# mit-han-lab/litepose

Measured on AMD Instinct MI355X. Metric: images/sec end-to-end (backbone+deconv+AE-group), LitePose-XS@256 b64, higher is better.
Workload: dtype f32

## Files before the change

### include/litepose_amd.h

```cpp
#ifndef LITEPOSE_AMD_H
#define LITEPOSE_AMD_H

#include <stddef.h>
#include <stdint.h>

#ifdef __cplusplus
extern "C" {
#endif

typedef enum lp_status {
    LP_OK = 0,
    LP_ERR_INVALID_ARG = -1,
    LP_ERR_UNKNOWN_KEY = -2,
    LP_ERR_SHAPE = -3,
    LP_ERR_MISSING_WEIGHT = -4,
    LP_ERR_NOT_FINALIZED = -5,
    LP_ERR_WORKSPACE = -6,
    LP_ERR_HIP = -7,
    LP_ERR_UNSUPPORTED = -8,
    LP_ERR_CAPACITY = -9
} lp_status;

const char* lp_last_error(void);
const char* lp_version(void);
// ... 221 lines not shown
                      float push_factor, float pull_factor, const float* d_g_heat, const float* d_g_push,
                      const float* d_g_pull, float* d_grad, void* stream);

size_t lp_bn_workspace_bytes(int N, int C, int HW);
int lp_bn_forward(const float* d_x, const float* d_gamma, const float* d_beta, float* d_running, const float* d_res,
                  float* d_y, double* d_stat, int N, int C, int HW, int act, int training, double momentum, double eps,
                  void* d_workspace, size_t workspace_bytes, void* stream);
int lp_bn_backward(const float* d_grad_y, const float* d_x, const float* d_gamma, const float* d_beta, const double* d_stat,
                   float* d_grad_x, float* d_grad_gamma, float* d_grad_beta, int N, int C, int HW, int act,
                   void* d_workspace, size_t workspace_bytes, void* stream);

#define LP_BN_SYNC_MAX_WORLD 64
int lp_bn_sync_stats(const float* d_x, int N, int C, int HW, double* d_row, void* d_workspace, size_t workspace_bytes,
                     void* stream);
int lp_bn_sync_forward(const float* d_x, const float* d_gamma, const float* d_beta, float* d_running, const float* d_res,
                       float* d_y, double* d_stat, const double* d_rows, int W, int N, int C, int HW, int act,
                       double momentum, double eps, void* stream);
int lp_bn_sync_backward_stats(const float* d_grad_y, const float* d_x, const float* d_gamma, const float* d_beta,
                              const double* d_stat, int N, int C, int HW, int act, double* d_row, void* d_workspace,
                              size_t workspace_bytes, void* stream);
int lp_bn_sync_backward(const float* d_grad_y, const float* d_x, const float* d_gamma, const float* d_beta,
                        const double* d_stat, const double* d_rows, int W, int rank, int N, int C, int HW, int act,
                        float* d_grad_x, float* d_grad_gamma, float* d_grad_beta, void* stream);

int lp_pw_tile_choice(int N, int Ca, int Cb, int Cout, int HW, int has_res);
#define LP_PW_WGRAD_SLICE 1024

#define LP_MBT_NONE 0
#define LP_MBT_TILE 1
#define LP_MBT_STRIP 2
#define LP_MBT_S2 3
int lp_mbt_form(int N, int Cin, int Cexp, int Cout, int H, int W, int K, int S, int has_res, int mode, int mode_s2,
                int mode_strip, int cus);
size_t lp_pw_forward_workspace_bytes(int Cin, int Cout);
int lp_pw_forward(const float* d_x, const float* d_w, float* d_y, int N, int Cin, int Cout, int HW, void* d_workspace,
                  size_t workspace_bytes, void* stream);
size_t lp_pw_backward_workspace_bytes(int N, int Cin, int Cout, int HW, int want_x, int want_w);
int lp_pw_backward(const float* d_grad_y, const float* d_x, const float* d_w, float* d_grad_x, float* d_grad_w, int N,
                   int Cin, int Cout, int HW, void* d_workspace, size_t workspace_bytes, void* stream);

#define LP_DW_WGRAD_SLICE 8
size_t lp_dw_forward_workspace_bytes(int C, int K);
int lp_dw_forward(const float* d_x, const float* d_w, float* d_y, int N, int C, int H, int W, int K, int S,
                  void* d_workspace, size_t workspace_bytes, void* stream);
size_t lp_dw_backward_workspace_bytes(int N, int C, int H, int W, int K, int S, int want_w);
int lp_dw_backward(const float* d_grad_y, const float* d_x, const float* d_w, float* d_grad_x, float* d_grad_w, int N,
                   int C, int H, int W, int K, int S, void* d_workspace, size_t workspace_bytes, void* stream);

#define LP_STEM_WGRAD_SLICE 2048
int lp_stem_forward(const float* d_x, const float* d_w, float* d_y, int N, int H, int W, void* stream);
size_t lp_stem_backward_workspace_bytes(int N, int H, int W);
int lp_stem_backward(const float* d_grad_y, const float* d_x, float* d_grad_w, int N, int H, int W, void* d_workspace,
                     size_t workspace_bytes, void* stream);

#define LP_DECONV_WGRAD_SLICE 1024
size_t lp_deconv_forward_workspace_bytes(int Ca, int Cb, int Cout);
int lp_deconv_forward(const float* d_xa, const float* d_wa, const float* d_xb, const float* d_wb, float* d_y, int N,
                      int Ca, int Cb, int Cout, int h, int w, void* d_workspace, size_t workspace_bytes, void* stream);
size_t lp_deconv_backward_workspace_bytes(int N, int Ca, int Cb, int Cout, int h, int w, int want_x, int want_w);
int lp_deconv_backward(const float* d_grad_y, const float* d_xa, const float* d_wa, const float* d_xb, const float* d_wb,
                       float* d_grad_xa, float* d_grad_xb, float* d_grad_wa, float* d_grad_wb, int N, int Ca,
                       int Cb, int Cout, int h, int w, void* d_workspace, size_t workspace_bytes, void* stream);

#define LP_CONV_WGRAD_SLICE 1024
size_t lp_conv_workspace_bytes(int N, int Ca, int Cb, int Cout, int H, int W, int K, int S, int ups);
int lp_conv_forward(const float* d_xa, const float* d_wa, const float* d_xb, const float* d_wb, const float* d_bias,
// ... 61 lines not shown
```

### litepose_amd/_native.py

```python
import ctypes as C
import os

import torch

_HERE = os.path.dirname(os.path.abspath(__file__))
LIB_PATH = os.path.join(_HERE, 'lib', 'liblitepose_amd.so')
if os.environ.get('LP_NATIVE_FLAVOUR'):
    LIB_PATH = os.path.join(_HERE, 'lib', 'liblitepose_amd_%s.so' % os.environ['LP_NATIVE_FLAVOUR'])

LP_MAX_STAGES, LP_MAX_BLOCKS, LP_MAX_DECONV = 8, 32, 4


class LpArch(C.Structure):
    _fields_ = [
        ('input_channel', C.c_int32), ('num_stages', C.c_int32),
        ('num_blocks', C.c_int32 * LP_MAX_STAGES), ('stride', C.c_int32 * LP_MAX_STAGES),
        ('channel', C.c_int32 * LP_MAX_STAGES),
        ('expand', (C.c_int32 * LP_MAX_BLOCKS) * LP_MAX_STAGES),
        ('kernel', (C.c_int32 * LP_MAX_BLOCKS) * LP_MAX_STAGES),
        ('num_deconv', C.c_int32), ('deconv_filters', C.c_int32 * LP_MAX_DECONV),
        ('head_channels', C.c_int32 * LP_MAX_DECONV),
        ('plain_head', C.c_int32),
        ('family', C.c_int32),
        ('upconv_kernel', C.c_int32),
# ... 103 lines not shown
                            vp, vp, vp, sz, vp]),
    'lp_kpt_eval': (i32, [vp, vp, vp, i32, i32, i32, i32, i32, vp, vp, vp, vp, vp, vp, i32, C.POINTER(C.c_double),
                          C.POINTER(C.c_double), i32, C.POINTER(C.c_double), i32, i32, vp, vp, vp, vp, vp, vp, vp]),
    'lp_draw_poses': (i32, [vp, i32, i32, i32, vp, vp, i32, i32, i32, C.POINTER(C.c_int32), i32,
                            C.POINTER(C.c_uint8), i32, i32, i32, vp]),
    'lp_draw_poses_v': (i32, [vp, sz, vp, i32, vp, vp, i32, i32, i32, C.POINTER(C.c_int32), i32,
                              C.POINTER(C.c_uint8), i32, i32, i32, vp]),
    'lp_draw_pass_prims': (i32, []),
    'lp_preprocess': (i32, [vp, i32, i32, C.POINTER(C.c_double), i32, i32, C.POINTER(C.c_float),
                            C.POINTER(C.c_float), vp, vp, vp]),
    'lp_preprocess_batch': (i32, [vp, i32, i32, i32, C.POINTER(C.c_double), i32, i32, C.POINTER(C.c_float),
                                  C.POINTER(C.c_float), vp, vp, vp]),
    'lp_warp_invert': (i32, [C.POINTER(C.c_double), C.POINTER(C.c_double)]),
    'lp_preprocess_batch_v': (i32, [vp, sz, vp, i32, i32, i32, C.POINTER(C.c_float), C.POINTER(C.c_float), vp, vp,
                                    vp]),
    'lp_augment_batch_v': (i32, [vp, sz, vp, i32, i32, i32, C.POINTER(C.c_float), C.POINTER(C.c_float), vp, vp, vp]),
    'lp_target_maps': (i32, [vp, i64, vp, vp, i32, i32, i32, C.POINTER(C.c_int32), vp, i32, C.c_double, i32, i32, vp, vp,
                             vp]),
    'lp_target_masks': (i32, [vp, sz, vp, i32, i32, vp, vp]),
    'lp_pose_loss_workspace_bytes': (sz, [i32, i32, i32]),
    'lp_pose_loss': (i32, [vp, i32, i32, i32, i32, i32, vp, vp, vp, i32, i32, C.c_float, C.c_float, C.c_float, vp, vp, vp,
                           vp, sz, vp]),
    'lp_pose_loss_grad': (i32, [vp, i32, i32, i32, i32, i32, vp, vp, vp, i32, i32, C.c_float, C.c_float, C.c_float, vp, vp,
                                vp, vp, vp]),
    'lp_bn_workspace_bytes': (sz, [i32, i32, i32]),
    'lp_bn_forward': (i32, [vp, vp, vp, vp, vp, vp, vp, i32, i32, i32, i32, i32, C.c_double, C.c_double, vp, sz, vp]),
    'lp_bn_backward': (i32, [vp, vp, vp, vp, vp, vp, vp, vp, i32, i32, i32, i32, vp, sz, vp]),
    'lp_bn_sync_stats': (i32, [vp, i32, i32, i32, vp, vp, sz, vp]),
    'lp_bn_sync_forward': (i32, [vp, vp, vp, vp, vp, vp, vp, vp, i32, i32, i32, i32, i32, C.c_double, C.c_double, vp]),
    'lp_bn_sync_backward_stats': (i32, [vp, vp, vp, vp, vp, i32, i32, i32, i32, vp, vp, sz, vp]),
    'lp_bn_sync_backward': (i32, [vp, vp, vp, vp, vp, vp, i32, i32, i32, i32, i32, i32, vp, vp, vp, vp]),
    'lp_pw_tile_choice': (i32, [i32, i32, i32, i32, i32, i32]),
    'lp_mbt_form': (i32, [i32] * 13),
    'lp_pw_forward_workspace_bytes': (sz, [i32, i32]),
    'lp_pw_forward': (i32, [vp, vp, vp, i32, i32, i32, i32, vp, sz, vp]),
    'lp_pw_backward_workspace_bytes': (sz, [i32, i32, i32, i32, i32, i32]),
    'lp_pw_backward': (i32, [vp, vp, vp, vp, vp, i32, i32, i32, i32, vp, sz, vp]),
    'lp_dw_forward_workspace_bytes': (sz, [i32, i32]),
    'lp_dw_forward': (i32, [vp, vp, vp, i32, i32, i32, i32, i32, i32, vp, sz, vp]),
    'lp_dw_backward_workspace_bytes': (sz, [i32, i32, i32, i32, i32, i32, i32]),
    'lp_dw_backward': (i32, [vp, vp, vp, vp, vp, i32, i32, i32, i32, i32, i32, vp, sz, vp]),
    'lp_stem_forward': (i32, [vp, vp, vp, i32, i32, i32, vp]),
    'lp_stem_backward_workspace_bytes': (sz, [i32, i32, i32]),
    'lp_stem_backward': (i32, [vp, vp, vp, i32, i32, i32, vp, sz, vp]),
    'lp_deconv_forward_workspace_bytes': (sz, [i32, i32, i32]),
    'lp_deconv_forward': (i32, [vp, vp, vp, vp, vp, i32, i32, i32, i32, i32, i32, vp, sz, vp]),
    'lp_deconv_backward_workspace_bytes': (sz, [i32, i32, i32, i32, i32, i32, i32, i32]),
    'lp_deconv_backward': (i32, [vp, vp, vp, vp, vp, vp, vp, vp, vp, i32, i32, i32, i32, i32, i32, vp, sz, vp]),
    'lp_conv_workspace_bytes': (sz, [i32] * 9),
    'lp_conv_forward': (i32, [vp, vp, vp, vp, vp, vp] + [i32] * 9 + [vp, sz, vp]),
    'lp_conv_backward': (i32, [vp] * 10 + [i32] * 9 + [vp, sz, vp]),
    'lp_optim_launches': (i32, [i32, C.POINTER(i64)]),
    'lp_optim_adam': (i32, [i32, C.POINTER(vp), C.POINTER(vp), C.POINTER(vp), C.POINTER(vp), C.POINTER(i64), vp, vp,
                            C.c_double, C.c_double, C.c_double, C.c_double, vp]),
    'lp_optim_sgd': (i32, [i32, C.POINTER(vp), C.POINTER(vp), C.POINTER(vp), C.POINTER(i64), vp, C.c_double, C.c_double,
                           i32, vp]),
    'lp_subnet_gather': (i32, [vp, i32, vp, i64, vp]),
    'lp_subnet_scatter_grad': (i32, [vp, i32, vp, i64, vp, i64, vp]),
    'lp_train_resize': (i32, [vp, vp, i32, i32, i32, i32, i32, i32, i32, C.POINTER(C.c_int32), C.POINTER(vp), C.POINTER(vp),
                              C.POINTER(vp), C.POINTER(vp), C.POINTER(vp), C.POINTER(vp), vp]),
    'lp_stream_abort_capture': (i32, [vp]),
    'lp_final_preds': (i32, [vp, vp, i32, i32, i32, i32, C.POINTER(C.c_double), C.POINTER(C.c_double),
                             i32, i32, vp]),
    'lp_final_preds_coef': (i32, [C.POINTER(C.c_double), C.POINTER(C.c_double), i32, i32, C.POINTER(C.c_double)]),
    'lp_final_preds_v': (i32, [vp, vp, i32, i32, i32, i32, vp, vp]),
}
# ... 38 lines not shown
```

### litepose_amd/csrc/engine.cpp

```cpp
#include <hip/hip_runtime.h>

#include <cmath>
#include <cstdio>
#include <cstdint>
#include <cstring>
#include <map>
#include <string>
#include <vector>

#include "../../include/litepose_amd.h"
#include "kernels.h"
#include "plan.h"

using namespace lp_plan;

namespace {

thread_local std::string g_err;
int fail(int code, const std::string& msg) {
    g_err = msg;
    return code;
}
#define HIP_OK(expr)                                                                   \
    do {                                                                               \
// ... 3 lines not shown
    } while (0)

static_assert(ACT_NONE == lp::ACT_NONE && ACT_RELU == lp::ACT_RELU && ACT_RELU6 == lp::ACT_RELU6, "plan.h restates lp::Act");

const char* storage_name(const Net* n) { return n->storage == LP_STORAGE_F16 ? "f16" : "bf16"; }

}

struct lp_net : lp_plan::Net {
    bool finalized = false;
    float* d_weights = nullptr;
    std::vector<char*> last_buf;
    int lastN = 0, lastH = 0, lastW = 0;
    bool profiling = false;
    std::vector<hipEvent_t> events;
    struct ProfEntry { std::string name, kernel; int64_t bytes, flops; int ev0, ev1; int64_t flops_valu; lp::LaunchNote launch; };
    std::vector<ProfEntry> prof_entries;
    int prof_ev = 0;
    static constexpr int MAX_SIDE = 8;
    hipStream_t side[MAX_SIDE] = {};
    hipEvent_t ev_fork = nullptr, ev_join[MAX_SIDE] = {};
    int nstreams = 0;
    int opt_mb16 = 1;
    int opt_mb16_run = 1;
    int opt_mb16_min = 48;
    int opt_mbt = 1, opt_mbt_s2 = 1;
    int opt_mbt_strip = 1;
    int opt_mbconv2 = 1;
    int opt_mbtb = 1, opt_mbtb_s2 = 1;
    int opt_pw3d = 1;
    int opt_mbtd = 1;
    int opt_headb = 1;
    int opt_headfuse = 1;
    int opt_dwt = 2;
    int opt_stem = 1;
    int opt_diag_dwpw = 0;
    struct OptEntryT { const char* key; int lo, hi; int lp_net::*field; };
    static const std::vector<OptEntryT>& options();
    std::vector<char> last_stored;
    struct CalibLayer { std::string bn; int C, div; size_t off; };
    struct Calib {
        lp_net* raw = nullptr;
        std::vector<CalibLayer> layers;
        std::map<std::string, int> index;
        std::vector<float> h_bn;
        float* d_bn = nullptr;
        double momentum = 0.1;
        int64_t steps = 0;
        bool uploaded = false;
    };
    Calib* calib = nullptr;
};

namespace {

size_t buf_elems(const lp_net* n, int b, int N, int H, int W, size_t esz) {
    const int d = n->bufs.div[b];
    const size_t f = (size_t)N * n->bufs.ch[b] * (H / d) * (W / d), q = 256 / esz;
    return (f + q - 1) / q * q;
}
size_t buf_floats(const lp_net* n, int b, int N, int H, int W) { return buf_elems(n, b, N, H, W, sizeof(float)); }

size_t buf_bytes(const lp_net* n, int b, int N, int H, int W) {
    const size_t esz = n->storage != LP_STORAGE_F32 ? sizeof(uint16_t) : sizeof(float);
    return buf_elems(n, b, N, H, W, esz) * esz;
}
// ... 327 lines not shown
}

int rule_dwpw3(const Part& c, size_t i) {
    const lp_net* n = c.n;
    const Op& o = n->ops[i];
    if (!(o.type == OP_DW && o.K == 3 && o.S == 1 && o.act == lp::ACT_RELU6 && i + 1 < n->ops.size())) return 0;
    const Op& pw = n->ops[i + 1];
    if (!(pw.type == OP_PW && pw.inA == o.out && pw.inB < 0 && pw.res < 0 && pw.act == lp::ACT_NONE && pw.has_bias)) return 0;
    const Planes pl = planes(c, o);
    const float* Wt = c.Wt;
    return lp::launch_dwpw(c.f(o.inA), Wt + o.w_off, Wt + o.b_off, Wt + pw.w_off, Wt + pw.b_off, nullptr, c.f(pw.out), c.NB,
                           o.Ca, pl.ih, pl.iw, o.K, o.S, pw.Cout, c.s, n->opt_diag_dwpw) ? 2 : 0;
}

int rule_head(const Part& c, size_t i) {
    const lp_net* n = c.n;
    const std::vector<Op>& ops = n->ops;
    const Op& o = ops[i];
    if (!(n->opt_headfuse && o.type == OP_DW && o.S == 1 && o.act == lp::ACT_RELU && i + 1 < ops.size())) return 0;
    const Op& a = ops[i + 1];
    const Op *d2 = nullptr, *pw = nullptr;
    if (o.K == 5 && a.type == OP_PW && a.inA == o.out && a.inB < 0 && a.res < 0 && a.act == lp::ACT_NONE &&
        (a.out == n->out0_buf || a.out == n->out1_buf))
        pw = &a;
    else if (i + 2 < ops.size() && a.type == OP_DW && ops[i + 2].type == OP_PW && ops[i + 2].inA == o.out &&
             ops[i + 2].inB == a.out && a.S == 1 && o.K == a.K && a.act == lp::ACT_RELU)
        d2 = &a, pw = &ops[i + 2];
    else
        return 0;
    const Planes pl = planes(c, o);
    const float* Wt = c.Wt;
    if (!lp::launch_headfuse(c.f(o.inA), o.Ca, d2 ? c.f(d2->inA) : nullptr, d2 ? d2->Ca : 0,
                             o.wpair_off ? Wt + o.wpair_off : nullptr, d2 && d2->wpair_off ? Wt + d2->wpair_off : nullptr,
                             Wt + pw->w_off, c.f(pw->out), c.NB, pl.oh, pl.ow, o.K, pw->Cout, c.s))
        return 0;
    return d2 ? 3 : 2;
}

const Rule F32_RULES[] = {{rule_mb16, block_name, nullptr}, {rule_mbt, block_name, nullptr}, {rule_stem3, stem_name, nullptr},
                          {rule_dwpw3, dwpw3_name, nullptr}, {rule_head, head_name, nullptr}};

int launch_op_f32(const Part& c, size_t i) {
    const lp_net* n = c.n;
    const Op& o = n->ops[i];
    const Planes pl = planes(c, o);
    const int ih = pl.ih, iw = pl.iw, oh = pl.oh, ow = pl.ow, NB = c.NB;
    const float* Wt = c.Wt;
    hipStream_t s = c.s;
    switch (o.type) {
        case OP_STEM:
            lp::launch_stem(c.x, Wt + o.w_off, Wt + o.b_off, c.f(o.out), NB, c.H, c.W, c.flip_from, c.x_batch, s);
            break;
        case OP_DW:
            lp::launch_dw(c.f(o.inA), Wt + o.w_off, Wt + o.wdup_off, Wt + o.b_off, c.f(o.out), NB, o.Ca, ih, iw, o.K, o.S,
                          o.act, s);
            break;
        case OP_PW:
            lp::launch_pw(c.f(o.inA), o.Ca, o.inB >= 0 ? c.f(o.inB) : nullptr, o.Cb, Wt + o.w_off,
                          o.has_bias ? Wt + o.b_off : nullptr, o.res >= 0 ? c.f(o.res) : nullptr, c.f(o.out), NB, oh * ow,
                          o.Cout, o.act, s, o.ws_off ? Wt + o.ws_off : nullptr, n->opt_pw3d);
            break;
        case OP_DECONV: {
            float* inB = o.inB >= 0 ? c.f(o.inB) : nullptr;
            if (o.w3_off && deconv4_enabled() && o.w4_off &&
                lp::launch_deconv4x3(c.f(o.inA), o.Ca, inB, o.Cb, Wt + o.w4_off, Wt + o.b3_off, c.f(o.out), NB, ih, iw,
                                     o.Cout, s)) {
            } else if (o.w3_off && deconv4_enabled())
// ... 418 lines not shown
        n->storage = storage;
        n->finalized = false;
        n->last_buf.clear();
    }
    return LP_OK;
}

int lp_net_get_storage(const lp_net* n) { return n ? n->storage : LP_ERR_INVALID_ARG; }

int lp_round16(const float* h_src, float* h_dst, int64_t count, int storage) {
    if ((!h_src || !h_dst) && count > 0) return fail(LP_ERR_INVALID_ARG, "null argument");
    if (storage != LP_STORAGE_BF16 && storage != LP_STORAGE_F16)
        return fail(LP_ERR_INVALID_ARG, "storage must be LP_STORAGE_BF16 or LP_STORAGE_F16");
    for (int64_t i = 0; i < count; ++i) h_dst[i] = round16(storage, h_src[i]);
    return LP_OK;
}

typedef lp_net::OptEntryT OptEntry;
const std::vector<OptEntry>& lp_net::options() {
    static const std::vector<OptEntry> t = {
        {"mb16", 0, 1, &lp_net::opt_mb16},
        {"mb16_run", 0, 1, &lp_net::opt_mb16_run},
        {"mb16_min", 0, 65536, &lp_net::opt_mb16_min},
        {"mbt", 0, 3, &lp_net::opt_mbt},
        {"mbt_s2", 0, 1, &lp_net::opt_mbt_s2},
        {"mbt_strip", 0, 2, &lp_net::opt_mbt_strip},
        {"mbconv2", 0, 1, &lp_net::opt_mbconv2},
        {"mbtb", 0, 1, &lp_net::opt_mbtb},
        {"mbtb_s2", 0, 1, &lp_net::opt_mbtb_s2},
        {"mbtd", 0, 1, &lp_net::opt_mbtd},
        {"pw3d", 0, 2, &lp_net::opt_pw3d},
        {"headb", 0, 1, &lp_net::opt_headb},
        {"headfuse", 0, 1, &lp_net::opt_headfuse},
        {"dwt", 0, 2, &lp_net::opt_dwt},
        {"stem", 0, 1, &lp_net::opt_stem},
        {"diag_dwpw", 0, 2, &lp_net::opt_diag_dwpw},
    };
    return t;
}

int lp_net_set_option(lp_net* n, const char* key, int value) {
    if (!n || !key) return fail(LP_ERR_INVALID_ARG, "null argument");
    for (const OptEntry& e : lp_net::options())
        if (!strcmp(key, e.key)) {
            if (value < e.lo || value > e.hi) return fail(LP_ERR_INVALID_ARG, std::string("option ") + key + ": value out of range");
#ifndef LP_DIAG_BUILD
            if (e.field == &lp_net::opt_diag_dwpw && value != 0)
                return fail(LP_ERR_UNSUPPORTED, "option diag_dwpw: the self-checking dwpw_kernel exists only in the diagnostics "
                                                "flavour of the library (python -m litepose_amd.build --flavour diag, "
                                                "LP_NATIVE_FLAVOUR=diag)");
#endif
            n->*(e.field) = value;
            return LP_OK;
        }
    return fail(LP_ERR_UNKNOWN_KEY, std::string("unknown option ") + key);
}

int lp_net_get_option(const lp_net* n, const char* key) {
    if (!n || !key) return fail(LP_ERR_INVALID_ARG, "null argument");
    for (const OptEntry& e : lp_net::options())
        if (!strcmp(key, e.key)) return n->*(e.field);
    return fail(LP_ERR_UNKNOWN_KEY, std::string("unknown option ") + key);
}

int lp_diag_read(uint32_t* h_words, int cap_words, int clear) {
    const int n = lp::dwpw_diag_read(h_words, cap_words, clear != 0);
// ... 66 lines not shown
```

### litepose_amd/csrc/kernels.h

```cpp
#pragma once
#include <hip/hip_runtime.h>
#include <stdint.h>

namespace lp {

enum Act { ACT_NONE = 0, ACT_RELU = 1, ACT_RELU6 = 2 };

bool uses_scratch(const void* kernel_fn);

bool kernel_ready(const void* kernel_fn, size_t dyn_lds);
bool kernel_allow_lds(const void* kernel_fn, size_t dyn_lds);

extern thread_local const char* last_kernel_tag;

struct LaunchNote { int grid = 0, block = 0, lds = 0, wgs_per_cu = 0; };
extern thread_local LaunchNote last_launch;
extern thread_local bool launch_notes;
void note_launch(const void* fn, dim3 grid, dim3 block, size_t lds);
#define LP_LAUNCH(kern, grid, block, lds, stream, ...)                                                   \
    do {                                                                                                 \
        if (lp::launch_notes) lp::note_launch(reinterpret_cast<const void*>(kern), grid, block, lds);    \
        hipLaunchKernelGGL(kern, grid, block, lds, stream, __VA_ARGS__);                                 \
    } while (0)

#ifdef LP_CLAIM_CU
#define LP_OWN_CU() asm volatile("; own the CU: whole register budget, no co-resident waves" ::: "v255")
#else
#define LP_OWN_CU() ((void)0)
#endif

void launch_stem(const float* x, const float* w, const float* b, float* out,
                 int N, int H, int W, int flip_from, int x_batch, hipStream_t s);

bool launch_stem3(const float* x, const float* w0t, const float* b0, const float* w1t, const float* b1,
                  const float* w2t, const float* b2, float* out, int N, int H, int W, int c0, int flip_from,
                  int x_batch, hipStream_t s);

bool launch_stem3b(const float* x, const float* w0t, const float* b0, const float* w1t, const float* b1,
                   const float* w2t, const float* b2, void* out, int N, int H, int W, int c0, int flip_from,
                   int x_batch, hipStream_t s, bool f16 = false);

void launch_dw(const float* in, const float* w, const float* wdup, const float* b, float* out,
               int N, int C, int H, int W, int K, int S, int act, hipStream_t s);

void launch_pw(const float* inA, int Ca, const float* inB, int Cb,
               const float* wp, const float* b, const float* res, float* out,
               int N, int HW, int Cout, int act, hipStream_t s, const void* wsplit = nullptr, int pw3d_mode = 1);
struct PwTile { int NB, PXV; };
PwTile pw_tile_choice(int N, int Ca, int Cb, int Cout, int HW, bool has_res);

bool launch_dwpw(const float* in, const float* wdw, const float* bdw, const float* wp, const float* bias,
                 const float* res, float* out, int N, int C, int H, int W, int K, int S, int Cout,
                 hipStream_t s, int diag = 0);
int dwpw_diag_read(unsigned* host, int cap_words, bool clear);

bool launch_headfuse(const float* inA, int Ca, const float* inB, int Cb, const float* wpairA, const float* wpairB,
                     const float* wp, float* out, int N, int H, int W, int K, int Cout, hipStream_t s);

bool launch_mbconv(const float* x, const float* w1p, const float* b1f, const float* wdw,
                   const float* bdw, const float* w2p, const float* b2f, const float* res, float* out,
                   int N, int Cin, int Cexp, int Cout, int H, int W, int K, int S, hipStream_t s,
                   const float* wdw_pair = nullptr, const void* w1_split = nullptr, const void* wdw_rows = nullptr,
                   int mbconv2 = 1);

constexpr int MB16_MAX_RUN = 10;
struct Mb16Run {
    const void* w1s[MB16_MAX_RUN];
    const float* b1f[MB16_MAX_RUN];
    const void* wrow[MB16_MAX_RUN];
    const void* w2s[MB16_MAX_RUN];
    const float* b2f[MB16_MAX_RUN];
    float* out[MB16_MAX_RUN];
    int nblocks;
};
bool mb16_supported(int Cin, int Cexp, int Cout, int H, int W, int K, int S, bool res);
bool launch_mb16(const float* x, const Mb16Run& run, bool res, int N, int Cin, int Cexp, int Cout, int H, int W,
                 int K, int S, hipStream_t s);

bool launch_mbt(const float* x, const void* w1s, const float* b1f, const void* wrow, const void* w2s,
                const float* b2f, const float* res, float* out, int N, int Cin, int Cexp, int Cout, int H, int W,
                int K, int S, hipStream_t s, int mode = 1, int mode_s2 = 1, int mode_strip = 1);
enum MbtKind { MBT_NONE = 0, MBT_TILE = 1, MBT_STRIP = 2, MBT_S2 = 3 };
struct MbtForm { int kind = MBT_NONE, CK = 0, NMT = 0; bool RES = false; };
MbtForm mbt_form(int N, int Cin, int Cexp, int Cout, int H, int W, int K, int S, bool has_res, int mode, int mode_s2,
                 int mode_strip, int cus);

void launch_deconv_pair(const float* inA, int Ca, const float* inB, int Cb,
                        const float* w, const float* b, float* out,
                        int N, int h, int w_, int Cout, hipStream_t s);

// ... 215 lines not shown
```

### litepose_amd/csrc/layer_api.cpp

```cpp
#include <hip/hip_runtime.h>

#include "../../include/litepose_amd.h"
#include "kernels.h"

extern "C" void lp_set_error_(const char* msg);

namespace {
int fail(int code, const char* msg) {
    lp_set_error_(msg);
    return code;
}
bool al16(const void* p) { return ((uintptr_t)p & 15) == 0; }
bool big(long long v) { return v > 0x7fffff00LL; }
size_t frag_floats(int M, int K) { return (size_t)((M + 31) / 32) * ((K + 1) / 2) * 64; }
size_t bias_floats(int M) { return (size_t)((M + 31) / 32) * 32; }
bool dw_shape_ok(int K, int S) { return (K == 3 || K == 5 || K == 7) && (S == 1 || S == 2); }
}

extern "C" {

size_t lp_bn_workspace_bytes(int N, int C, int HW) {
    if (N < 1 || C < 1 || HW < 1 || C > 65535 || big((long long)N * HW) || big((long long)C * HW)) return 0;
    return lp::bn_partial_doubles(N, C, HW) * sizeof(double);
}
// ... 98 lines not shown
                        const double* d_stat, const double* d_rows, int W, int rank, int N, int C, int HW, int act,
                        float* d_grad_x, float* d_grad_gamma, float* d_grad_beta, void* stream) {
    if (int rc = sync_check(N, C, HW, act, W, rank)) return rc;
    if (!d_grad_y || !d_x || !d_gamma || !d_beta || !d_stat || !d_rows || !d_grad_x || !d_grad_gamma || !d_grad_beta)
        return fail(LP_ERR_INVALID_ARG, "null argument");
    if (!al16(d_grad_y) || !al16(d_x) || !al16(d_grad_x) || !al8(d_stat) || !al8(d_rows))
        return fail(LP_ERR_INVALID_ARG, "grad_y, x and grad_x must be 16-byte, stat and rows 8-byte aligned");
    lp::launch_bn_sync_bwd(d_grad_y, d_x, d_gamma, d_beta, d_stat, d_rows, W, rank, d_grad_x, d_grad_gamma,
                           d_grad_beta, N, C, HW, act, (hipStream_t)stream);
    if (hipGetLastError() != hipSuccess) return fail(LP_ERR_HIP, "bn_sync_backward launch failed");
    return LP_OK;
}

static int pw_check(int N, int Cin, int Cout, int HW) {
    if (N < 1 || Cin < 1 || Cout < 1 || HW < 1) return fail(LP_ERR_INVALID_ARG, "N, Cin, Cout and HW must be positive");
    if (Cin > 65535 || Cout > 65535 || big((long long)N * HW) || big((long long)Cin * HW) || big((long long)Cout * HW))
        return fail(LP_ERR_UNSUPPORTED, "channels must be <= 65535, N * HW and C * HW at most 2^31 - 256");
    return LP_OK;
}

int lp_pw_tile_choice(int N, int Ca, int Cb, int Cout, int HW, int has_res) {
    if (N < 1 || Ca < 1 || Cb < 0 || Cout < 1 || HW < 1) return fail(LP_ERR_INVALID_ARG, "N, Ca, Cout and HW must be positive, Cb non-negative");
    const lp::PwTile t = lp::pw_tile_choice(N, Ca, Cb, Cout, HW, has_res != 0);
    return t.NB * 16 + t.PXV;
}

int lp_mbt_form(int N, int Cin, int Cexp, int Cout, int H, int W, int K, int S, int has_res, int mode, int mode_s2,
                int mode_strip, int cus) {
    if (N < 1 || Cin < 1 || Cexp < 1 || Cout < 1 || H < 1 || W < 1 || K < 1 || S < 1)
        return fail(LP_ERR_INVALID_ARG, "N, Cin, Cexp, Cout, H, W, K and S must be positive");
    const lp::MbtForm f = lp::mbt_form(N, Cin, Cexp, Cout, H, W, K, S, has_res != 0, mode, mode_s2, mode_strip, cus);
    if (f.kind == lp::MBT_NONE) return LP_MBT_NONE;
    return f.kind + 16 * f.CK + 256 * f.NMT + (f.RES ? 4096 : 0);
}

size_t lp_pw_forward_workspace_bytes(int Cin, int Cout) {
    if (Cin < 1 || Cout < 1 || Cin > 65535 || Cout > 65535) return 0;
    return (frag_floats(Cout, Cin) + bias_floats(Cout)) * sizeof(float);
}

int lp_pw_forward(const float* d_x, const float* d_w, float* d_y, int N, int Cin, int Cout, int HW, void* d_workspace,
                  size_t workspace_bytes, void* stream) {
    if (int rc = pw_check(N, Cin, Cout, HW)) return rc;
    if (!d_x || !d_w || !d_y) return fail(LP_ERR_INVALID_ARG, "null argument");
    if (!al16(d_x) || !al16(d_y)) return fail(LP_ERR_INVALID_ARG, "x and y must be 16-byte aligned");
    if (!d_workspace || workspace_bytes < lp_pw_forward_workspace_bytes(Cin, Cout)) return fail(LP_ERR_WORKSPACE, "pw workspace too small");
    if (!al16(d_workspace)) return fail(LP_ERR_WORKSPACE, "pw workspace must be 16-byte aligned");
    hipStream_t s = (hipStream_t)stream;
    float* wp = (float*)d_workspace;
    float* zb = wp + frag_floats(Cout, Cin);
    lp::launch_pw_pack(d_w, Cout, Cin, false, wp, zb, s);
    lp::launch_pw(d_x, Cin, nullptr, 0, wp, zb, nullptr, d_y, N, HW, Cout, lp::ACT_NONE, s);
    if (hipGetLastError() != hipSuccess) return fail(LP_ERR_HIP, "pw_forward launch failed");
    return LP_OK;
}

size_t lp_pw_backward_workspace_bytes(int N, int Cin, int Cout, int HW, int want_x, int want_w) {
    if (N < 1 || Cin < 1 || Cout < 1 || HW < 1 || Cin > 65535 || Cout > 65535 || big((long long)N * HW)) return 0;
    size_t fl = 0;
    if (want_x) fl += frag_floats(Cin, Cout) + bias_floats(Cin);
    if (want_w) fl += (size_t)lp::pw_wgrad_slices((long)N * HW) * Cout * Cin;
    return fl * sizeof(float);
}

int lp_pw_backward(const float* d_grad_y, const float* d_x, const float* d_w, float* d_grad_x, float* d_grad_w, int N,
                   int Cin, int Cout, int HW, void* d_workspace, size_t workspace_bytes, void* stream) {
// ... 328 lines not shown
```

### litepose_amd/csrc/net_kernels.hip

```cpp
#include "kernels.h"
#include "fused_common.h"
#include "split3.h"

#include <cstdio>
#include <cstdlib>
#include <type_traits>
#include <utility>

namespace lp {

thread_local const char* last_kernel_tag = "";
thread_local LaunchNote last_launch;
thread_local bool launch_notes = false;

void note_launch(const void* fn, dim3 grid, dim3 block, size_t lds) {
    int per_cu = 0;
    const int threads = (int)(block.x * block.y * block.z);
    if (hipOccupancyMaxActiveBlocksPerMultiprocessor(&per_cu, fn, threads, lds) != hipSuccess) per_cu = 0;
    last_launch.grid = (int)((long)grid.x * grid.y * grid.z);
    last_launch.block = threads;
    last_launch.lds = (int)lds;
    last_launch.wgs_per_cu = per_cu;
}

// ... 1269 lines not shown
        const unsigned z = 0;
        if (hipMemcpyToSymbol(HIP_SYMBOL(lp_dwpw_diag_log), &z, 4, 0, hipMemcpyHostToDevice) != hipSuccess) return -1;
    }
    return (int)n;
#endif
}

bool launch_dwpw(const float* in, const float* wdw, const float* bdw, const float* wp, const float* bias,
                 const float* res, float* out, int N, int C, int H, int W, int K, int S, int Cout,
                 hipStream_t s, int diag) {
    if ((K != 7 && K != 3) || (C & 31) || (W & 3) || Cout > 96) return false;
    if (K == 3 && (S != 1 || Cout > 32)) return false;
    {
        const int OHt = (H + 2 * (K / 2) - K) / S + 1, OWt = (W + 2 * (K / 2) - K) / S + 1;
        if ((long)OHt * OWt < 4096) return false;
    }
    const int nb = (Cout + 31) / 32;
    if (K == 3) {
        launch_dwpw_t<3, 1, 1>(in, wdw, bdw, wp, bias, res, out, N, C, H, W, Cout, s, diag);
        return true;
    }
#define LP_F(SV, NBV) launch_dwpw_t<7, SV, NBV>(in, wdw, bdw, wp, bias, res, out, N, C, H, W, Cout, s)
    if (S == 1) { if (nb == 1) LP_F(1, 1); else if (nb == 2) LP_F(1, 2); else LP_F(1, 3); }
    else { if (nb == 1) LP_F(2, 1); else if (nb == 2) LP_F(2, 2); else LP_F(2, 3); }
#undef LP_F
    return true;
}


__device__ __forceinline__ int quad_row_of_lane(int lane) {
    return (int)((0xFDCE5764B98A1320ull >> (4 * (lane >> 2))) & 15);
}

template <int NB, bool DUAL>
__global__ __launch_bounds__(256) void headfuse_kernel(const float* __restrict__ inA, int Ca,
                                                       const float* __restrict__ inB, int Cb,
                                                       const float* __restrict__ wpairA,
                                                       const float* __restrict__ wpairB,
                                                       const float* __restrict__ wp,
                                                       float* __restrict__ out, int H, int W, int tilesX, int tilesY,
                                                       int Cout, int xcd_remap) {
    constexpr int K = 5;
    constexpr int HALO = K / 2;
    constexpr int IH = 16 + K - 1;
    constexpr int QPR = 6;
    constexpr int RS = 13;
    constexpr int TILE_SLOTS = IH * RS;
    extern __shared__ __attribute__((aligned(16))) float smem[];
    const int C = DUAL ? Ca + Cb : Ca;
    float* slab = smem;
    const int lane = threadIdx.x & 63;
    const int wave = __builtin_amdgcn_readfirstlane(threadIdx.x >> 6);
    f32x4* tile = reinterpret_cast<f32x4*>(smem + 16 * 256) + wave * TILE_SLOTS;
    const int unit = xcd_remap ? xcd_contiguous_id(blockIdx.x, gridDim.x) : blockIdx.x;
    const int tq = unit / tilesX;
    const int tx = unit - tq * tilesX;
    const int n = tq / tilesY;
    const int ty = tq - n * tilesY;
    const int ix0 = tx * 16 - 4, iy0 = ty * 16 - HALO;
    constexpr int NQ = IH * QPR, NLD = (NQ + 63) / 64;
    const int row = quad_row_of_lane(lane), strip = lane & 3;
    const int half = lane >> 5, pl = lane & 31;
    const int KP = C >> 1;
    const int cblocks = (Cout + 31) >> 5;
    int st_off[NLD], st_lds[NLD];
#pragma unroll
    for (int i = 0; i < NLD; ++i) {
        const int e = lane + 64 * i;
        const int r = e / QPR, q = e - r * QPR;
        const int iy = iy0 + r, ix = ix0 + 4 * q;
        const bool ok = e < NQ && iy >= 0 && iy < H && ix >= 0 && ix < W;
        st_off[i] = ok ? iy * W + ix : -1;
        st_lds[i] = e < NQ ? r * RS + 2 * q : -1;
    }
    const long HW = (long)H * W;
    const float* imgA = inA + (long)n * Ca * HW;
    const float* imgB = DUAL ? inB + (long)n * Cb * HW : imgA;
    float afr[NB][32];
#pragma unroll
    for (int i = 0; i < NB; ++i)
#pragma unroll
        for (int kp = 0; kp < 32; ++kp)
            afr[i][kp] = wp[((long)min(i, cblocks - 1) * KP + min(kp, KP - 1)) * 64 + lane];
    f32x4 pre[2][NLD];
    auto issue = [&](int cp) {
        const int c = 2 * cp;
        const float* plane = (!DUAL || c < Ca) ? imgA + (long)c * HW : imgB + (long)(c - Ca) * HW;
#pragma unroll
        for (int h2 = 0; h2 < 2; ++h2)
#pragma unroll
            for (int i = 0; i < NLD; ++i) {
                f32x4 v = *reinterpret_cast<const f32x4*>(plane + h2 * HW + max(st_off[i], 0));
                if (st_off[i] < 0) v = f32x4{0.f, 0.f, 0.f, 0.f};
                pre[h2][i] = v;
            }
    };
    issue(wave);
    f32x16 acc[NB][2];
#pragma unroll
    for (int i = 0; i < NB; ++i)
#pragma unroll
        for (int v = 0; v < 2; ++v)
#pragma unroll
            for (int r = 0; r < 16; ++r) acc[i][v][r] = 0.f;
    const float* bsrc = slab + half * 256 + wave * 64 + 2 * pl;
    auto kpair_mfma = [&](int kp) {
        const f32x2 bv = *reinterpret_cast<const f32x2*>(bsrc + (kp & 7) * 512);
#pragma unroll
        for (int i = 0; i < NB; ++i) {
            acc[i][0] = __builtin_amdgcn_mfma_f32_32x32x2f32(afr[i][kp], bv[0], acc[i][0], 0, 0, 0);
            acc[i][1] = __builtin_amdgcn_mfma_f32_32x32x2f32(afr[i][kp], bv[1], acc[i][1], 0, 0, 0);
        }
    };
    const int NR = (KP + 3) >> 2;
#pragma unroll
    for (int u = 0; u < 8; ++u) {
        if (u >= NR) break;
        const int cp = wave + 4 * u;
        const bool has = cp < KP;
        const int c = 2 * cp;
        f32x2 dacc[4];
        f32x2 dbias = {0.f, 0.f};
        const float* wc = wpairA;
        if (has) {
#pragma unroll
            for (int i = 0; i < NLD; ++i)
                if (st_lds[i] >= 0) {
                    const f32x4 a = pre[0][i], b = pre[1][i];
                    tile[st_lds[i]] = f32x4{a[0], b[0], a[1], b[1]};
                    tile[st_lds[i] + 1] = f32x4{a[2], b[2], a[3], b[3]};
                }
            __builtin_amdgcn_fence(__ATOMIC_RELEASE, "wavefront");
            __builtin_amdgcn_wave_barrier();
            __builtin_amdgcn_fence(__ATOMIC_ACQUIRE, "wavefront");
            if (cp + 4 < KP) issue(cp + 4);
            wc = (!DUAL || c < Ca) ? wpairA + (long)cp * (K * K + 1) * 2 : wpairB + (long)(cp - (Ca >> 1)) * (K * K + 1) * 2;
            dbias = f32x2{wc[2 * K * K], wc[2 * K * K + 1]};
#pragma unroll
            for (int i = 0; i < 4; ++i) dacc[i] = DUAL ? dbias : f32x2{0.f, 0.f};
        }
#pragma unroll
        for (int ky = 0; ky < K; ++ky) {
            if (has) {
                const f32x4* lr = tile + (row + ky) * RS + 2 * strip;
                f32x2 v[12];
#pragma unroll
                for (int q = 0; q < 6; ++q) {
                    const f32x4 tt = lr[q];
                    v[2 * q] = f32x2{tt[0], tt[1]};
                    v[2 * q + 1] = f32x2{tt[2], tt[3]};
                }
#pragma unroll
                for (int kx = 0; kx < K; ++kx) {
                    const f32x2 w2 = {wc[2 * (ky * K + kx)], wc[2 * (ky * K + kx) + 1]};
#pragma unroll
                    for (int i = 0; i < 4; ++i) dacc[i] = __builtin_elementwise_fma(v[(4 - HALO) + kx + i], w2, dacc[i]);
                }
            }
            if (u > 0 && ky < 4) {
                const int kp = 4 * (u - 1) + ky;
                if (kp < KP) {
                    __builtin_amdgcn_sched_barrier(0);
                    kpair_mfma(kp);
                    __builtin_amdgcn_sched_barrier(0);
                }
            }
        }
        if (has) {
            f32x4 o0, o1;
#pragma unroll
            for (int i = 0; i < 4; ++i) {
                o0[i] = fmaxf(DUAL ? dacc[i][0] : dacc[i][0] + dbias[0], 0.f);
                o1[i] = fmaxf(DUAL ? dacc[i][1] : dacc[i][1] + dbias[1], 0.f);
            }
            *reinterpret_cast<f32x4*>(slab + (2 * (cp & 7)) * 256 + row * 16 + strip * 4) = o0;
            *reinterpret_cast<f32x4*>(slab + (2 * (cp & 7) + 1) * 256 + row * 16 + strip * 4) = o1;
        }
        __syncthreads();
    }
#pragma unroll
    for (int u = 0; u < 8; ++u)
        if (u == NR - 1) {
#pragma unroll
            for (int j = 0; j < 4; ++j)
                if (4 * u + j < KP) kpair_mfma(4 * u + j);
        }
    const int p0 = wave * 64 + 2 * pl;
    const int oy = ty * 16 + (p0 >> 4), ox = tx * 16 + (p0 & 15);
    if (oy >= H || ox >= W) return;
#pragma unroll
    for (int i = 0; i < NB; ++i) {
        if (i >= cblocks) break;
        const int cob = i * 32 + 4 * half;
#pragma unroll
        for (int r = 0; r < 16; ++r) {
            const int co = cob + (r & 3) + 8 * (r >> 2);
            if (co < Cout)
                *reinterpret_cast<f32x2*>(out + ((long)n * Cout + co) * HW + (long)oy * W + ox) =
                    f32x2{acc[i][0][r], acc[i][1][r]};
        }
    }
}

bool launch_headfuse(const float* inA, int Ca, const float* inB, int Cb, const float* wpairA, const float* wpairB,
                     const float* wp, float* out, int N, int H, int W, int K, int Cout, hipStream_t s) {
    const int C = Ca + Cb;
    const bool dual = inB != nullptr;
    if (!wpairA || (dual ? (!wpairB || (Cb & 1)) : Cb != 0) || K != 5 || (Ca & 1) || C > 64 || (W & 15) || (H & 15) ||
        Cout > 64 || (long)H * W < 4096)
        return false;
    const int tilesX = W / 16, tilesY = H / 16;
    const int grid = N * tilesX * tilesY;
    const size_t lds = (size_t)(16 * 256 + 4 * (16 + 5 - 1) * 13 * 4) * sizeof(float);
    static_assert((16 * 256 + 4 * (16 + 5 - 1) * 13 * 4) * sizeof(float) <= 64 * 1024,
                  "33 KB: below the default dynamic-LDS limit, no per-device attribute call needed (ADVICE r05)");
    last_kernel_tag = "headfuse_kernel";
#define LP_HF(NBV, DV) LP_LAUNCH((headfuse_kernel<NBV, DV>), dim3(grid), dim3(256), lds, s, inA, Ca, inB, Cb, \
                                 wpairA, wpairB, wp, out, H, W, tilesX, tilesY, Cout, xcd_remap_mode())
    if (dual) { if (Cout <= 32) LP_HF(1, true); else LP_HF(2, true); }
    else { if (Cout <= 32) LP_HF(1, false); else LP_HF(2, false); }
#undef LP_HF
    return true;
}

constexpr int MB_RS = 24, MB_ROWS = 22, MB_PLANE = MB_RS * MB_ROWS;

constexpr int MB2_RS = 26, MB2_PAIR = MB_ROWS * MB2_RS * 2;

__device__ __forceinline__ int mb2_row_of_lane(int lane) {
    return (int)((0xFDCE5764B98A1320ull >> (4 * (lane >> 2))) & 15);
}

template <bool RES>
__global__ __launch_bounds__(256, 2) void mbconv_kernel(
    const float* __restrict__ x,
    const float* __restrict__ w1p,
    const float* __restrict__ b1f,
    const float* __restrict__ wdwp,
    const float* __restrict__ bdw,
    const float* __restrict__ w2p,
    const float* __restrict__ b2f,
    float* __restrict__ out,
    int Cin, int Cexp, int Cout, int H, int W, int tilesX, int tilesY, int xcd_remap) {
    extern __shared__ __attribute__((aligned(16))) float E[];
    const int lane = threadIdx.x & 63;
    const int wave = __builtin_amdgcn_readfirstlane(threadIdx.x >> 6);
    const int half = lane >> 5, pl = lane & 31;
    const int unit = xcd_remap ? xcd_contiguous_id(blockIdx.x, gridDim.x) : blockIdx.x;
    const int tq = unit / tilesX;
    const int tx = unit - tq * tilesX;
    const int n = tq / tilesY;
    const int ty = tq - n * tilesY;
    const int x0 = tx * 16, y0 = ty * 16;
// ... 1083 lines not shown
```

Before: 23610.

## Add block-layout depthwise path to fused head kernel with register row streaming

Adds a BLK variant of the fused head kernel. Each lane computes a 2x2 output block for one channel pair, streaming input rows from LDS into registers so each row load serves two output rows. The MFMA pointwise step is interleaved under every row, and the NB==1 case gets a higher occupancy bound. It is on by default and falls back to the old variant if the new one spills to scratch. In exchange it adds template instantiations, a different slab write pattern with a swizzle, and some register pressure risk.

```diff
diff --git a/include/litepose_amd.h b/include/litepose_amd.h
--- a/include/litepose_amd.h
+++ b/include/litepose_amd.h
@@ -277,6 +277,9 @@
 #define LP_MBT_S2 3
 int lp_mbt_form(int N, int Cin, int Cexp, int Cout, int H, int W, int K, int S, int has_res, int mode, int mode_s2,
                 int mode_strip, int cus);
+#define LP_HEADFUSE_NONE 0
+#define LP_HEADFUSE_BLK 16
+int lp_headfuse_form(int Ca, int Cb, int Cout, int H, int W, int K, int mode_blk);
 size_t lp_pw_forward_workspace_bytes(int Cin, int Cout);
 int lp_pw_forward(const float* d_x, const float* d_w, float* d_y, int N, int Cin, int Cout, int HW, void* d_workspace,
                   size_t workspace_bytes, void* stream);
diff --git a/litepose_amd/_native.py b/litepose_amd/_native.py
--- a/litepose_amd/_native.py
+++ b/litepose_amd/_native.py
@@ -159,6 +159,7 @@
     'lp_bn_sync_backward': (i32, [vp, vp, vp, vp, vp, vp, i32, i32, i32, i32, i32, i32, vp, vp, vp, vp]),
     'lp_pw_tile_choice': (i32, [i32, i32, i32, i32, i32, i32]),
     'lp_mbt_form': (i32, [i32] * 13),
+    'lp_headfuse_form': (i32, [i32] * 7),
     'lp_pw_forward_workspace_bytes': (sz, [i32, i32]),
     'lp_pw_forward': (i32, [vp, vp, vp, i32, i32, i32, i32, vp, sz, vp]),
     'lp_pw_backward_workspace_bytes': (sz, [i32, i32, i32, i32, i32, i32]),
diff --git a/litepose_amd/csrc/engine.cpp b/litepose_amd/csrc/engine.cpp
--- a/litepose_amd/csrc/engine.cpp
+++ b/litepose_amd/csrc/engine.cpp
@@ -59,6 +59,7 @@
     int opt_mbtd = 1;
     int opt_headb = 1;
     int opt_headfuse = 1;
+    int opt_head_blk = 1;
     int opt_dwt = 2;
     int opt_stem = 1;
     int opt_diag_dwpw = 0;
@@ -452,7 +453,7 @@
     const float* Wt = c.Wt;
     if (!lp::launch_headfuse(c.f(o.inA), o.Ca, d2 ? c.f(d2->inA) : nullptr, d2 ? d2->Ca : 0,
                              o.wpair_off ? Wt + o.wpair_off : nullptr, d2 && d2->wpair_off ? Wt + d2->wpair_off : nullptr,
-                             Wt + pw->w_off, c.f(pw->out), c.NB, pl.oh, pl.ow, o.K, pw->Cout, c.s))
+                             Wt + pw->w_off, c.f(pw->out), c.NB, pl.oh, pl.ow, o.K, pw->Cout, c.s, n->opt_head_blk))
         return 0;
     return d2 ? 3 : 2;
 }
@@ -937,6 +938,7 @@
         {"pw3d", 0, 2, &lp_net::opt_pw3d},
         {"headb", 0, 1, &lp_net::opt_headb},
         {"headfuse", 0, 1, &lp_net::opt_headfuse},
+        {"head_blk", 0, 1, &lp_net::opt_head_blk},
         {"dwt", 0, 2, &lp_net::opt_dwt},
         {"stem", 0, 1, &lp_net::opt_stem},
         {"diag_dwpw", 0, 2, &lp_net::opt_diag_dwpw},
diff --git a/litepose_amd/csrc/kernels.h b/litepose_amd/csrc/kernels.h
--- a/litepose_amd/csrc/kernels.h
+++ b/litepose_amd/csrc/kernels.h
@@ -55,7 +55,9 @@
 int dwpw_diag_read(unsigned* host, int cap_words, bool clear);
 
 bool launch_headfuse(const float* inA, int Ca, const float* inB, int Cb, const float* wpairA, const float* wpairB,
-                     const float* wp, float* out, int N, int H, int W, int K, int Cout, hipStream_t s);
+                     const float* wp, float* out, int N, int H, int W, int K, int Cout, hipStream_t s, int mode_blk);
+struct HeadForm { int NB = 0; bool blk = false; };
+HeadForm headfuse_form(int Ca, int Cb, bool dual, int Cout, int H, int W, int K, int mode_blk);
 
 bool launch_mbconv(const float* x, const float* w1p, const float* b1f, const float* wdw,
                    const float* bdw, const float* w2p, const float* b2f, const float* res, float* out,
diff --git a/litepose_amd/csrc/layer_api.cpp b/litepose_amd/csrc/layer_api.cpp
--- a/litepose_amd/csrc/layer_api.cpp
+++ b/litepose_amd/csrc/layer_api.cpp
@@ -154,6 +154,14 @@
     const lp::MbtForm f = lp::mbt_form(N, Cin, Cexp, Cout, H, W, K, S, has_res != 0, mode, mode_s2, mode_strip, cus);
     if (f.kind == lp::MBT_NONE) return LP_MBT_NONE;
     return f.kind + 16 * f.CK + 256 * f.NMT + (f.RES ? 4096 : 0);
+}
+
+int lp_headfuse_form(int Ca, int Cb, int Cout, int H, int W, int K, int mode_blk) {
+    if (Ca < 1 || Cb < 0 || Cout < 1 || H < 1 || W < 1 || K < 1)
+        return fail(LP_ERR_INVALID_ARG, "Ca, Cout, H, W and K must be positive, Cb non-negative");
+    const lp::HeadForm f = lp::headfuse_form(Ca, Cb, Cb > 0, Cout, H, W, K, mode_blk);
+    if (f.NB == 0) return LP_HEADFUSE_NONE;
+    return f.NB + (f.blk ? LP_HEADFUSE_BLK : 0);
 }
 
 size_t lp_pw_forward_workspace_bytes(int Cin, int Cout) {
diff --git a/litepose_amd/csrc/net_kernels.hip b/litepose_amd/csrc/net_kernels.hip
--- a/litepose_amd/csrc/net_kernels.hip
+++ b/litepose_amd/csrc/net_kernels.hip
@@ -1325,8 +1325,12 @@
     return (int)((0xFDCE5764B98A1320ull >> (4 * (lane >> 2))) & 15);
 }
 
-template <int NB, bool DUAL>
-__global__ __launch_bounds__(256) void headfuse_kernel(const float* __restrict__ inA, int Ca,
+__device__ __forceinline__ int quad_block_of_lane(int lane) {
+    return (int)((0xFD579B31EC468A20ull >> (4 * (lane >> 2))) & 15);
+}
+
+template <int NB, bool DUAL, bool BLK>
+__global__ __launch_bounds__(256, (BLK && NB == 1) ? 4 : 1) void headfuse_kernel(const float* __restrict__ inA, int Ca,
                                                        const float* __restrict__ inB, int Cb,
                                                        const float* __restrict__ wpairA,
                                                        const float* __restrict__ wpairB,
@@ -1353,6 +1357,8 @@
     const int ix0 = tx * 16 - 4, iy0 = ty * 16 - HALO;
     constexpr int NQ = IH * QPR, NLD = (NQ + 63) / 64;
     const int row = quad_row_of_lane(lane), strip = lane & 3;
+    const int qb = quad_block_of_lane(lane);
+    const int rp = qb & 7, cpair = 4 * (qb >> 3) + (lane & 3);
     const int half = lane >> 5, pl = lane & 31;
     const int KP = C >> 1;
     const int cblocks = (Cout + 31) >> 5;
@@ -1403,6 +1409,14 @@
         for (int i = 0; i < NB; ++i) {
             acc[i][0] = __builtin_amdgcn_mfma_f32_32x32x2f32(afr[i][kp], bv[0], acc[i][0], 0, 0, 0);
             acc[i][1] = __builtin_amdgcn_mfma_f32_32x32x2f32(afr[i][kp], bv[1], acc[i][1], 0, 0, 0);
+        }
+    };
+    auto mfma_under_row = [&](int u, int R) {
+        const int kp = 4 * (u - 1) + R;
+        if (u > 0 && R < 4 && (BLK || kp < KP)) {
+            __builtin_amdgcn_sched_barrier(0);
+            kpair_mfma(kp);
+            __builtin_amdgcn_sched_barrier(0);
         }
     };
     const int NR = (KP + 3) >> 2;
@@ -1427,47 +1441,103 @@
             __builtin_amdgcn_wave_barrier();
             __builtin_amdgcn_fence(__ATOMIC_ACQUIRE, "wavefront");
             if (cp + 4 < KP) issue(cp + 4);
-            wc = (!DUAL || c < Ca) ? wpairA + (long)cp * (K * K + 1) * 2 : wpairB + (long)(cp - (Ca >> 1)) * (K * K + 1) * 2;
+            if constexpr (!BLK) {
+                wc = (!DUAL || c < Ca) ? wpairA + (long)cp * (K * K + 1) * 2 : wpairB + (long)(cp - (Ca >> 1)) * (K * K + 1) * 2;
+                dbias = f32x2{wc[2 * K * K], wc[2 * K * K + 1]};
+#pragma unroll
+                for (int i = 0; i < 4; ++i) dacc[i] = DUAL ? dbias : f32x2{0.f, 0.f};
+            }
+        }
+        if constexpr (BLK) {
+            const int cpw = has ? cp : 0;
+            wc = (!DUAL || 2 * cpw < Ca) ? wpairA + (long)cpw * (K * K + 1) * 2 : wpairB + (long)(cpw - (Ca >> 1)) * (K * K + 1) * 2;
             dbias = f32x2{wc[2 * K * K], wc[2 * K * K + 1]};
 #pragma unroll
             for (int i = 0; i < 4; ++i) dacc[i] = DUAL ? dbias : f32x2{0.f, 0.f};
-        }
-#pragma unroll
-        for (int ky = 0; ky < K; ++ky) {
+            const f32x4* lr = tile + 2 * rp * RS + cpair + 1;
+            {
+                f32x4 rn[3], rc[3];
+#pragma unroll
+                for (int t = 0; t < 3; ++t) rn[t] = lr[t];
+#pragma unroll
+                for (int R = 0; R < K + 1; ++R) {
+#pragma unroll
+                    for (int t = 0; t < 3; ++t) { rc[t] = rn[t]; keep_b128(rc[t]); }
+                    __builtin_amdgcn_sched_barrier(0);
+                    if (R < K) {
+#pragma unroll
+                        for (int t = 0; t < 3; ++t) rn[t] = lr[(R + 1) * RS + t];
+                    }
+                    __builtin_amdgcn_sched_barrier(0);
+                    const f32x2 P[6] = {{rc[0][0], rc[0][1]}, {rc[0][2], rc[0][3]}, {rc[1][0], rc[1][1]},
+                                        {rc[1][2], rc[1][3]}, {rc[2][0], rc[2][1]}, {rc[2][2], rc[2][3]}};
+                    if (R >= 1) {
+#pragma unroll
+                        for (int kx = 0; kx < K; ++kx) {
+                            const f32x2 w2 = {wc[2 * ((R - 1) * K + kx)], wc[2 * ((R - 1) * K + kx) + 1]};
+#pragma unroll
+                            for (int i = 0; i < 2; ++i) dacc[2 + i] = __builtin_elementwise_fma(P[kx + i], w2, dacc[2 + i]);
+                        }
+                    }
+                    if (R < K) {
+#pragma unroll
+                        for (int kx = 0; kx < K; ++kx) {
+                            const f32x2 w2 = {wc[2 * (R * K + kx)], wc[2 * (R * K + kx) + 1]};
+#pragma unroll
+                            for (int i = 0; i < 2; ++i) dacc[i] = __builtin_elementwise_fma(P[kx + i], w2, dacc[i]);
+                        }
+                    }
+                    mfma_under_row(u, R);
+                }
+            }
+            {
+                f32x2 o[2][2];
+#pragma unroll
+                for (int ch = 0; ch < 2; ++ch)
+#pragma unroll
+                    for (int a = 0; a < 2; ++a)
+#pragma unroll
+                        for (int i = 0; i < 2; ++i)
+                            o[ch][a][i] = fmaxf(DUAL ? dacc[2 * a + i][ch] : dacc[2 * a + i][ch] + dbias[ch], 0.f);
+                const int swp = (rp >> 1) & 1;
+                float* sb = (has ? slab + (2 * (cp & 7)) * 256 : reinterpret_cast<float*>(tile)) + 2 * rp * 16 + 2 * cpair;
+#pragma unroll
+                for (int ch = 0; ch < 2; ++ch) {
+                    *reinterpret_cast<f32x2*>(sb + ch * 256 + 16 * swp) = swp ? o[ch][1] : o[ch][0];
+                    *reinterpret_cast<f32x2*>(sb + ch * 256 + 16 * (swp ^ 1)) = swp ? o[ch][0] : o[ch][1];
+                }
+            }
+        } else {
+#pragma unroll
+            for (int ky = 0; ky < K; ++ky) {
+                if (has) {
+                    const f32x4* lr = tile + (row + ky) * RS + 2 * strip;
+                    f32x2 v[12];
+#pragma unroll
+                    for (int q = 0; q < 6; ++q) {
+                        const f32x4 tt = lr[q];
+                        v[2 * q] = f32x2{tt[0], tt[1]};
+                        v[2 * q + 1] = f32x2{tt[2], tt[3]};
+                    }
+#pragma unroll
+                    for (int kx = 0; kx < K; ++kx) {
+                        const f32x2 w2 = {wc[2 * (ky * K + kx)], wc[2 * (ky * K + kx) + 1]};
+#pragma unroll
+                        for (int i = 0; i < 4; ++i) dacc[i] = __builtin_elementwise_fma(v[(4 - HALO) + kx + i], w2, dacc[i]);
+                    }
+                }
+                mfma_under_row(u, ky);
+            }
             if (has) {
-                const f32x4* lr = tile + (row + ky) * RS + 2 * strip;
-                f32x2 v[12];
-#pragma unroll
-                for (int q = 0; q < 6; ++q) {
-                    const f32x4 tt = lr[q];
-                    v[2 * q] = f32x2{tt[0], tt[1]};
-                    v[2 * q + 1] = f32x2{tt[2], tt[3]};
-                }
-#pragma unroll
-                for (int kx = 0; kx < K; ++kx) {
-                    const f32x2 w2 = {wc[2 * (ky * K + kx)], wc[2 * (ky * K + kx) + 1]};
-#pragma unroll
-                    for (int i = 0; i < 4; ++i) dacc[i] = __builtin_elementwise_fma(v[(4 - HALO) + kx + i], w2, dacc[i]);
-                }
-            }
-            if (u > 0 && ky < 4) {
-                const int kp = 4 * (u - 1) + ky;
-                if (kp < KP) {
-                    __builtin_amdgcn_sched_barrier(0);
-                    kpair_mfma(kp);
-                    __builtin_amdgcn_sched_barrier(0);
-                }
-            }
-        }
-        if (has) {
-            f32x4 o0, o1;
-#pragma unroll
-            for (int i = 0; i < 4; ++i) {
-                o0[i] = fmaxf(DUAL ? dacc[i][0] : dacc[i][0] + dbias[0], 0.f);
-                o1[i] = fmaxf(DUAL ? dacc[i][1] : dacc[i][1] + dbias[1], 0.f);
-            }
-            *reinterpret_cast<f32x4*>(slab + (2 * (cp & 7)) * 256 + row * 16 + strip * 4) = o0;
-            *reinterpret_cast<f32x4*>(slab + (2 * (cp & 7) + 1) * 256 + row * 16 + strip * 4) = o1;
+                f32x4 o0, o1;
+#pragma unroll
+                for (int i = 0; i < 4; ++i) {
+                    o0[i] = fmaxf(DUAL ? dacc[i][0] : dacc[i][0] + dbias[0], 0.f);
+                    o1[i] = fmaxf(DUAL ? dacc[i][1] : dacc[i][1] + dbias[1], 0.f);
+                }
+                *reinterpret_cast<f32x4*>(slab + (2 * (cp & 7)) * 256 + row * 16 + strip * 4) = o0;
+                *reinterpret_cast<f32x4*>(slab + (2 * (cp & 7) + 1) * 256 + row * 16 + strip * 4) = o1;
+            }
         }
         __syncthreads();
     }
@@ -1495,23 +1565,42 @@
     }
 }
 
+HeadForm headfuse_form(int Ca, int Cb, bool dual, int Cout, int H, int W, int K, int mode_blk) {
+    HeadForm f;
+    if ((dual ? (Cb & 1) : Cb != 0) || K != 5 || (Ca & 1) || Ca + Cb > 64 || (W & 15) || (H & 15) || Cout > 64 ||
+        (long)H * W < 4096)
+        return f;
+    f.NB = Cout <= 32 ? 1 : 2;
+    f.blk = mode_blk != 0;
+    return f;
+}
+
 bool launch_headfuse(const float* inA, int Ca, const float* inB, int Cb, const float* wpairA, const float* wpairB,
-                     const float* wp, float* out, int N, int H, int W, int K, int Cout, hipStream_t s) {
-    const int C = Ca + Cb;
+                     const float* wp, float* out, int N, int H, int W, int K, int Cout, hipStream_t s, int mode_blk) {
     const bool dual = inB != nullptr;
-    if (!wpairA || (dual ? (!wpairB || (Cb & 1)) : Cb != 0) || K != 5 || (Ca & 1) || C > 64 || (W & 15) || (H & 15) ||
-        Cout > 64 || (long)H * W < 4096)
-        return false;
+    const HeadForm form = headfuse_form(Ca, Cb, dual, Cout, H, W, K, mode_blk);
+    if (!wpairA || (dual && !wpairB) || form.NB == 0) return false;
     const int tilesX = W / 16, tilesY = H / 16;
     const int grid = N * tilesX * tilesY;
     const size_t lds = (size_t)(16 * 256 + 4 * (16 + 5 - 1) * 13 * 4) * sizeof(float);
     static_assert((16 * 256 + 4 * (16 + 5 - 1) * 13 * 4) * sizeof(float) <= 64 * 1024,
                   "33 KB: below the default dynamic-LDS limit, no per-device attribute call needed (ADVICE r05)");
     last_kernel_tag = "headfuse_kernel";
-#define LP_HF(NBV, DV) LP_LAUNCH((headfuse_kernel<NBV, DV>), dim3(grid), dim3(256), lds, s, inA, Ca, inB, Cb, \
-                                 wpairA, wpairB, wp, out, H, W, tilesX, tilesY, Cout, xcd_remap_mode())
-    if (dual) { if (Cout <= 32) LP_HF(1, true); else LP_HF(2, true); }
-    else { if (Cout <= 32) LP_HF(1, false); else LP_HF(2, false); }
+#define LP_HF(NBV, DV, BV) \
+    do { \
+        if (BV && uses_scratch(reinterpret_cast<const void*>(&headfuse_kernel<NBV, DV, BV>))) \
+            LP_LAUNCH((headfuse_kernel<NBV, DV, false>), dim3(grid), dim3(256), lds, s, inA, Ca, inB, Cb, \
+                      wpairA, wpairB, wp, out, H, W, tilesX, tilesY, Cout, xcd_remap_mode()); \
+        else \
+            LP_LAUNCH((headfuse_kernel<NBV, DV, BV>), dim3(grid), dim3(256), lds, s, inA, Ca, inB, Cb, \
+                      wpairA, wpairB, wp, out, H, W, tilesX, tilesY, Cout, xcd_remap_mode()); \
+    } while (0)
+#define LP_HF_D(NBV, BV) do { if (dual) LP_HF(NBV, true, BV); else LP_HF(NBV, false, BV); } while (0)
+#define LP_HF_B(NBV) do { if (form.blk) LP_HF_D(NBV, true); else LP_HF_D(NBV, false); } while (0)
+    if (form.NB == 1) LP_HF_B(1);
+    else LP_HF_B(2);
+#undef LP_HF_B
+#undef LP_HF_D
 #undef LP_HF
     return true;
 }
```

New measurement: 23710, median of 6. Within noise of the previous version (+0.4%).
